# 1556174776/simple_pbft

Hardware: AMD Instinct MI355X
Metric: sig verifies/sec at 1/2/4/8 MI355X; p50 quorum-cert verify latency (higher is better)
Workload: dtype u32; 1 GPU; config4: 1048576 ECDSA-P256 sigs sharded N/1, 100-key table, 1% corrupted (8 classes); global_batch=1048576, keys=100, parallelism=shard1 (strong scaling: independent per-GPU shards, no collective), streams=2

## Files before the change

### simple_pbft_amd/csrc/kernels.h

```cpp
#pragma once
#include <hip/hip_runtime.h>
#include <stddef.h>
#include <stdint.h>

namespace pbftv {

size_t table_bytes(int w);
int table_windows(int w);
#define PBFTV_COMBOS_G29(X) X(29, 24) X(29, 22) X(29, 21) X(29, 20) X(29, 16)
#define PBFTV_COMBOS_G26(X) X(26, 24) X(26, 22) X(26, 21) X(26, 20) X(26, 16)
#define PBFTV_COMBOS_G24(X) X(24, 24) X(24, 22) X(24, 20) X(24, 16)
#define PBFTV_COMBOS_SMALL(X) X(20, 20) X(16, 16) X(16, 12) X(16, 8) X(8, 8)
#define PBFTV_COMBOS(X) PBFTV_COMBOS_G29(X) PBFTV_COMBOS_G26(X) PBFTV_COMBOS_G24(X) PBFTV_COMBOS_SMALL(X)
#define PBFTV_TABLE_WIDTHS(X) X(8) X(12) X(16) X(20) X(21) X(22) X(24) X(26) X(29)
struct TableScratch {
  void* bases;
  void* lbuf;
  void* hbuf;
  void* small_scratch;
  void* entry_scratch;
  uint64_t entry_lanes;
};
struct TableScratchSizes {
  size_t bases, lbuf, hbuf, small_scratch, entry_scratch;
  uint64_t entry_lanes;
};
TableScratchSizes table_scratch_sizes(int w, uint32_t nbases);
hipError_t launch_build_tables(int w, const uint32_t* keys_le, uint32_t key0, uint32_t nb, int with_g,
                               uint32_t* valid, uint32_t* const* tabs, TableScratch& sc, hipStream_t st);
size_t ecdsa_record_bytes(uint64_t n);
int scalar_batch(uint64_t n);
size_t scalar_prefix_bytes(uint64_t n);
struct KeyOrder {
  const uint32_t* total;
  uint32_t* claim;
  uint32_t nkeys;
};
hipError_t launch_ecdsa_scalars(const uint8_t* hashes, const uint8_t* sigs, const uint32_t* key_idx, uint64_t n,
                                const uint32_t* key_valid, uint32_t nkeys, void* rec, void* prefix,
                                const KeyOrder& ko, hipStream_t st);
hipError_t launch_ecdsa_comb(int wg, int wq, const void* rec, uint64_t n, const uint32_t* gtab,
                             const uint32_t* const* qtabs,
                             uint8_t* bitmap, uint8_t* okb, const uint32_t* cuflag, hipStream_t st);
constexpr uint32_t kCuFlagWords = 4096;
bool key_sort_wanted(uint64_t n, uint32_t nkeys);
size_t key_sort_header_bytes();
size_t key_sort_scratch_bytes(uint64_t n, uint32_t nkeys);
hipError_t launch_key_count(const uint32_t* key_idx, uint64_t n, uint32_t nkeys, void* scratch, uint32_t parity,
                            KeyOrder* out, hipStream_t st);
hipError_t launch_pack_bits(const uint8_t* okb, uint64_t n, uint8_t* bitmap, hipStream_t st);
struct CombArgs {
  const void* rec;
  uint64_t n;
  const uint32_t* gtab;
  const uint32_t* const* qtabs;
  uint8_t* bitmap;
  uint8_t* okb;
  const uint32_t* cuflag;
};
struct WaveArgs {
  const uint8_t* hashes;
  const uint8_t* sigs;
  const uint32_t* key_idx;
  uint64_t n;
  const uint32_t* key_valid;
  uint32_t nkeys;
  const uint32_t* gtab;
  const uint32_t* const* qtabs;
  uint8_t* bitmap;
  uint8_t* okbytes;
  bool one_wave;
};
hipError_t launch_ecdsa_wave(int wg, int wq, const uint8_t* hashes, const uint8_t* sigs, const uint32_t* key_idx,
                             uint64_t n, const uint32_t* key_valid, uint32_t nkeys, const uint32_t* gtab,
                             const uint32_t* const* qtabs, uint8_t* bitmap, uint8_t* okbytes, hipStream_t st,
                             bool one_wave = false);
uint64_t wave_path_max();
constexpr int kRowsExact = 4;

struct QcMail {
  uint32_t bell, n, stop, expired_s0, cap, halt, expired_s1, pad[9];
  static constexpr uint32_t kQcSlots = 8;
  static constexpr uint32_t kQcCap = 128;
  static constexpr int kArmSlots = 2;
  __host__ __device__ uint32_t* expired(int s) { return s ? &expired_s1 : &expired_s0; }
  static constexpr size_t slot_off(uint32_t i) { return 64 + 192 * (size_t)i; }
  static constexpr size_t live_off(int s = 0) { return 64 + 192 * (size_t)kQcSlots + 4 * (size_t)kQcCap * s; }
  static constexpr size_t res_off(uint32_t = kQcCap) { return live_off(kArmSlots); }
  static constexpr size_t arrays_off(uint32_t cap = kQcCap) {
    return (res_off() + (cap > kQcCap ? cap : kQcCap) + 63) & ~(size_t)63;
// ... 82 lines not shown
```

### simple_pbft_amd/csrc/p256_kernels.hip

```cpp
#include <hip/hip_runtime.h>

#include <cstdlib>

#include "kernels.h"
#include "verify_kernels.h"

namespace pbftv {

#ifndef PBFTV_SCAL_BLOCK_INV_MIN_K
#define PBFTV_SCAL_BLOCK_INV_MIN_K 4
#endif

#ifndef PBFTV_SCAL_WAVES
#define PBFTV_SCAL_WAVES 1
#endif

constexpr uint32_t kSortBlocks = 256;
constexpr uint32_t kSortMaxKeys = 1024;
constexpr uint32_t kSortHdr = kSortMaxKeys + 64;

template <int W>
struct TabGeom {
  using G = CombGeom<W>;
  static constexpr int CL = G::kEnt < 256 ? G::kEnt : (G::kW <= 16 ? 256 : 1 << (G::kW / 2));
// ... 245 lines not shown
  switch (w) {
#define PBFTV_W(W) \
  case W: return CombGeom<W>::kBytes;
    PBFTV_TABLE_WIDTHS(PBFTV_W)
#undef PBFTV_W
    default: return 0;
  }
}

int table_windows(int w) {
  switch (w) {
#define PBFTV_W(W) \
  case W: return CombGeom<W>::kWin;
    PBFTV_TABLE_WIDTHS(PBFTV_W)
#undef PBFTV_W
    default: return 0;
  }
}

hipError_t launch_build_tables(int w, const uint32_t* keys_le, uint32_t key0, uint32_t nb, int with_g,
                               uint32_t* valid, uint32_t* const* tabs, TableScratch& sc, hipStream_t st) {
  switch (w) {
#define PBFTV_W(W) \
  case W: return build_tables_w<W>(keys_le, key0, nb, with_g, valid, tabs, sc, st);
    PBFTV_TABLE_WIDTHS(PBFTV_W)
#undef PBFTV_W
    default: return hipErrorInvalidValue;
  }
}

__device__ __forceinline__ void block_key_hist(uint32_t* h, const uint32_t* __restrict__ key_idx, uint64_t n,
                                               uint32_t nkeys) {
  const uint32_t nb = nkeys + 1;
  for (uint32_t b = threadIdx.x; b < nb; b += blockDim.x) h[b] = 0;
  __syncthreads();
  const uint64_t chunk = (n + gridDim.x - 1) / gridDim.x, lo = (uint64_t)blockIdx.x * chunk;
  const uint64_t hi = lo + chunk < n ? lo + chunk : n;
  for (uint64_t i = lo + threadIdx.x; i < hi; i += blockDim.x) {
    const uint32_t k = key_idx[i];
    atomicAdd(&h[k < nkeys ? k : nkeys], 1u);
  }
  __syncthreads();
}

__global__ void __launch_bounds__(256) k_key_hist(const uint32_t* __restrict__ key_idx, uint64_t n, uint32_t nkeys,
                                                  uint32_t* __restrict__ cur, uint32_t* __restrict__ other) {
  __shared__ uint32_t h[kSortMaxKeys + 1];
  if (blockIdx.x == 0)
    for (uint32_t b = threadIdx.x; b < 2 * kSortHdr; b += blockDim.x) other[b] = 0;
  block_key_hist(h, key_idx, n, nkeys);
  for (uint32_t b = threadIdx.x; b <= nkeys; b += blockDim.x)
    if (h[b]) atomicAdd(&cur[b], h[b]);
}

__device__ __forceinline__ void block_key_starts(const uint32_t* __restrict__ total, uint32_t nkeys, uint32_t* start,
                                                 uint32_t* part) {
  constexpr uint32_t kPer = (kSortMaxKeys + 1 + 255) / 256;
  const uint32_t t = threadIdx.x, m = nkeys + 1;
  uint32_t v[kPer], sum = 0;
  PBFTV_UNROLL for (uint32_t k = 0; k < kPer; ++k) {
    const uint32_t b = kPer * t + k;
    v[k] = b < m ? total[b] : 0u;
    sum += v[k];
  }
  part[t] = sum;
  __syncthreads();
  for (uint32_t off = 1; off < 256; off <<= 1) {
    const uint32_t x = t >= off ? part[t - off] : 0u;
    __syncthreads();
    part[t] += x;
    __syncthreads();
  }
  uint32_t run = part[t] - sum;
  PBFTV_UNROLL for (uint32_t k = 0; k < kPer; ++k) {
    const uint32_t b = kPer * t + k;
    if (b < m) start[b] = run;
    run += v[k];
  }
  __syncthreads();
}

template <int K>
// ... 124 lines not shown
        if constexpr (kPre) {
          PBFTV_UNROLL for (int t = 0; t < 8; ++t) e[t] = pe[j][t];
        } else {
          load_be256(hashes + 32 * i, e);
        }
        fe ev, rv, t;
        fe_from_words(ev, e);
        fe_from_words(rv, r);
        fn_mul(t, ev, w);
        fn_canon(t, t);
        fe_to_words(u1, t);
        fn_mul(t, rv, w);
        fn_canon(t, t);
        fe_to_words(u2, t);
      }
      uint64_t at = i;
      uint32_t kj;
      if constexpr (kPre) kj = pk[j];
      else kj = key_idx[i];
      if (sorted) at = atomicAdd(&kh[kj < nk ? kj : nk], 1u);
      SigRec* o = rec + at;
      o->q[0] = make_uint4(u1[0], u1[1], u1[2], u1[3]);
      o->q[1] = make_uint4(u1[4], u1[5], u1[6], u1[7]);
      o->q[2] = make_uint4(u2[0], u2[1], u2[2], u2[3]);
      o->q[3] = make_uint4(u2[4], u2[5], u2[6], u2[7]);
      o->q[4] = make_uint4(r[0], r[1], r[2], r[3]);
      o->q[5] = make_uint4(r[4], r[5], r[6], r[7]);
      o->q[6] = make_uint4(ok ? kj : 0u, (uint32_t)i, ok ? 1u : 0u, 0u);
    }
  }
  PBFTV_SPROBE(5, okm);
}

__global__ void __launch_bounds__(256) k_pack_bits(const uint8_t* __restrict__ okb, uint64_t n,
                                                   uint8_t* __restrict__ bitmap) {
  const uint64_t b = (uint64_t)blockIdx.x * blockDim.x + threadIdx.x;
  if (8 * b >= n) return;
  uint32_t v = 0;
  if (8 * b + 8 <= n) {
    const uint2 w = *reinterpret_cast<const uint2*>(okb + 8 * b);
    PBFTV_UNROLL for (int k = 0; k < 4; ++k) v |= ((w.x >> (8 * k)) & 1u) << k;
    PBFTV_UNROLL for (int k = 0; k < 4; ++k) v |= ((w.y >> (8 * k)) & 1u) << (4 + k);
  } else {
    for (uint64_t k = 0; 8 * b + k < n; ++k) v |= (okb[8 * b + k] ? 1u : 0u) << k;
  }
  bitmap[b] = (uint8_t)v;
}

bool key_sort_wanted(uint64_t n, uint32_t nkeys) {
  if (const char* e = getenv("PBFTV_KEY_SORT")) {
    if (e[0] == '0') return false;
    if (e[0] == '1') return nkeys <= kSortMaxKeys && n < (1ull << 32);
  }
  return nkeys > 8 && nkeys <= kSortMaxKeys && n >= 32768 && n < (1ull << 32);
}

size_t key_sort_header_bytes() { return (size_t)(4 * kSortHdr) * 4; }
size_t key_sort_scratch_bytes(uint64_t, uint32_t) { return key_sort_header_bytes(); }

hipError_t launch_key_count(const uint32_t* key_idx, uint64_t n, uint32_t nkeys, void* scratch, uint32_t parity,
                            KeyOrder* out, hipStream_t st) {
  if (nkeys > kSortMaxKeys) return hipErrorInvalidValue;
  uint32_t* hdr = reinterpret_cast<uint32_t*>(scratch);
  uint32_t* cur = hdr + (parity & 1u) * 2 * kSortHdr;
  uint32_t* other = hdr + (~parity & 1u) * 2 * kSortHdr;
  *out = KeyOrder{cur, cur + kSortHdr, nkeys};
  if (n == 0) return hipSuccess;
  hipLaunchKernelGGL(k_key_hist, dim3(kSortBlocks), dim3(256), 0, st, key_idx, n, nkeys, cur, other);
  return hipGetLastError();
}

hipError_t launch_pack_bits(const uint8_t* okb, uint64_t n, uint8_t* bitmap, hipStream_t st) {
  if (n == 0) return hipSuccess;
  const uint64_t bytes = (n + 7) / 8;
  hipLaunchKernelGGL(k_pack_bits, dim3((uint32_t)((bytes + 255) / 256)), dim3(256), 0, st, okb, n, bitmap);
  return hipGetLastError();
}

bool launch_comb_part_g29(int wg, int wq, const CombArgs& a, hipStream_t st);
bool launch_comb_part_g26(int wg, int wq, const CombArgs& a, hipStream_t st);
bool launch_comb_part_g24(int wg, int wq, const CombArgs& a, hipStream_t st);
bool launch_comb_part_small(int wg, int wq, const CombArgs& a, hipStream_t st);
bool launch_wave_part_g29(int wg, int wq, const WaveArgs& a, hipStream_t st);
bool launch_wave_part_g26(int wg, int wq, const WaveArgs& a, hipStream_t st);
bool launch_wave_part_g24(int wg, int wq, const WaveArgs& a, hipStream_t st);
bool launch_wave_part_small(int wg, int wq, const WaveArgs& a, hipStream_t st);

hipError_t launch_ecdsa_wave(int wg, int wq, const uint8_t* hashes, const uint8_t* sigs, const uint32_t* key_idx,
                             uint64_t n, const uint32_t* key_valid, uint32_t nkeys, const uint32_t* gtab,
                             const uint32_t* const* qtabs, uint8_t* bitmap, uint8_t* okbytes, hipStream_t st,
                             bool one_wave) {
  if (n == 0) return hipSuccess;
  if (n > 0xFFFFFFFFull) return hipErrorInvalidValue;
  const WaveArgs a{hashes, sigs, key_idx, n, key_valid, nkeys, gtab, qtabs, bitmap, okbytes, one_wave};
  if (launch_wave_part_g29(wg, wq, a, st) || launch_wave_part_g26(wg, wq, a, st) ||
      launch_wave_part_g24(wg, wq, a, st) || launch_wave_part_small(wg, wq, a, st))
    return hipGetLastError();
  return hipErrorInvalidValue;
}

bool launch_armed_part_g29(int wg, int wq, const ArmArgs& a, hipStream_t st);
bool launch_armed_part_g26(int wg, int wq, const ArmArgs& a, hipStream_t st);
bool launch_armed_part_g24(int wg, int wq, const ArmArgs& a, hipStream_t st);
bool launch_armed_part_small(int wg, int wq, const ArmArgs& a, hipStream_t st);

hipError_t launch_ecdsa_wave_armed(int wg, int wq, const ArmArgs& a, hipStream_t st) {
  if (launch_armed_part_g29(wg, wq, a, st) || launch_armed_part_g26(wg, wq, a, st) ||
      launch_armed_part_g24(wg, wq, a, st) || launch_armed_part_small(wg, wq, a, st))
// ... 20 lines not shown
size_t scalar_prefix_bytes(uint64_t n) {
  const int k = scalar_batch(n);
  const uint64_t L = ((n + k - 1) / k + 255) / 256 * 256;
  return (size_t)k * 9 * L * 4;
}

template <int K>
static void launch_scalars_k(const uint8_t* hashes, const uint8_t* sigs, const uint32_t* key_idx, uint64_t n,
                             const uint32_t* key_valid, uint32_t nkeys, void* rec, uint32_t* prefix,
                             const KeyOrder& ko, hipStream_t st) {
  const uint64_t lanes = (n + K - 1) / K;
  const uint64_t blocks = (lanes + 255) / 256;
  hipLaunchKernelGGL(k_ecdsa_scalars<K>, dim3((uint32_t)blocks), dim3(256), 0, st, hashes, sigs, key_idx, n,
                     key_valid, nkeys, reinterpret_cast<SigRec*>(rec), prefix, ko);
}

hipError_t launch_ecdsa_scalars(const uint8_t* hashes, const uint8_t* sigs, const uint32_t* key_idx, uint64_t n,
                                const uint32_t* key_valid, uint32_t nkeys, void* rec, void* prefix,
                                const KeyOrder& ko, hipStream_t st) {
  if (n == 0) return hipSuccess;
  uint32_t* pf = reinterpret_cast<uint32_t*>(prefix);
  switch (scalar_batch(n)) {
    case 1: launch_scalars_k<1>(hashes, sigs, key_idx, n, key_valid, nkeys, rec, pf, ko, st); break;
    case 2: launch_scalars_k<2>(hashes, sigs, key_idx, n, key_valid, nkeys, rec, pf, ko, st); break;
    case 4: launch_scalars_k<4>(hashes, sigs, key_idx, n, key_valid, nkeys, rec, pf, ko, st); break;
    case 8: launch_scalars_k<8>(hashes, sigs, key_idx, n, key_valid, nkeys, rec, pf, ko, st); break;
    default: launch_scalars_k<16>(hashes, sigs, key_idx, n, key_valid, nkeys, rec, pf, ko, st); break;
  }
  return hipGetLastError();
}

hipError_t launch_ecdsa_comb(int wg, int wq, const void* rec, uint64_t n, const uint32_t* gtab,
                             const uint32_t* const* qtabs,
                             uint8_t* bitmap, uint8_t* okb, const uint32_t* cuflag, hipStream_t st) {
  if (n == 0) return hipSuccess;
  const CombArgs a{rec, n, gtab, qtabs, bitmap, okb, cuflag};
  if (launch_comb_part_g29(wg, wq, a, st) || launch_comb_part_g26(wg, wq, a, st) ||
      launch_comb_part_g24(wg, wq, a, st) || launch_comb_part_small(wg, wq, a, st))
    return hipGetLastError();
  return hipErrorInvalidValue;
}

size_t ecdsa_record_bytes(uint64_t n) { return (size_t)n * sizeof(SigRec); }

}

#ifdef PBFTV_SCAL_PROBE
extern "C" int pbftv_debug_scal_probe(uint64_t* out, size_t n) {
  return (int)hipMemcpyFromSymbol(out, HIP_SYMBOL(pbftv::g_scal_probe), n * sizeof(uint64_t), 0,
                                  hipMemcpyDeviceToHost);
}
#endif
```

### simple_pbft_amd/csrc/pbftv_api.cpp

```cpp
#include <hip/hip_runtime.h>

#include <algorithm>
#include <atomic>
#include <chrono>
#include <condition_variable>
#include <cstdio>
#include <cstdlib>
#include <cstring>
#include <functional>
#include <initializer_list>
#include <map>
#include <set>
#include <memory>
#include <mutex>
#include <string>
#include <thread>
#include <vector>

#include "../../include/pbftv.h"
#include "gojson.h"
#include "gojson_enc.h"
#include "kernels.h"

namespace {
// ... 107 lines not shown
  unsigned flags = hipHostMallocCoherent | hipHostMallocMapped;
  hipError_t ensure(size_t bytes) {
    if (bytes <= cap) return hipSuccess;
    if (p) {
      GpuQuiesce q(-1);
      (void)hipHostFree(p);
    }
    p = nullptr;
    cap = 0;
    size_t want = std::max<size_t>(bytes, 1 << 16);
    hipError_t e = hipHostMalloc(&p, want, flags);
    if (e == hipSuccess) cap = want;
    return e;
  }
  void release() {
    if (p) {
      GpuQuiesce q(-1);
      (void)hipHostFree(p);
    }
    p = nullptr;
    cap = 0;
  }
  HostBuf() = default;
  HostBuf(const HostBuf&) = delete;
  HostBuf& operator=(const HostBuf&) = delete;
  ~HostBuf() { release(); }
  template <class T>
  T* as() const {
    return reinterpret_cast<T*>(p);
  }
};

struct VerifyScratch {
  DevBuf rec, prefix, ksort, okb;
  uint32_t sort_parity = 0;
  void release() {
    rec.release();
    prefix.release();
    ksort.release();
    okb.release();
  }
};

struct Device {
  int id = -1;
  hipStream_t stream = nullptr;
  std::mutex mu;
  bool have_keys = false;
  bool mail_registered = false;
  bool keeper_stop = false, keeper_idle = false;
  bool qc_armed_served = false;
  HostBuf stage;
  std::atomic<uint32_t> arm_seq{0};
  uint32_t seq_counter = 0;
  int arm_stream = 1;
  uint32_t armed_first = 0;
  uint32_t retiring = 0;
  uint32_t arm_waves = 0;
  bool arm_wide = false;
  uint32_t qc_nmax = 0;
  uint32_t qc_nmax_prev = 0;
  uint32_t qc_slots = 4;
  uint32_t qc_wmax = 0;
  uint32_t qc_wslots = 0;
  bool arm_live = false;
  std::chrono::steady_clock::time_point last_wide{};
  std::chrono::steady_clock::time_point armed_at{}, last_qc{};
  uint64_t qc_ns_entry = 0, qc_ns_handover = 0, qc_ns_total = 0, qc_ns_slots = 0;
  char hot_end[1] = {};
  uint64_t qc_calls = 0, qc_armed = 0, qc_reruns = 0, qc_exact_sigs = 0, qc_launches = 0, qc_armings = 0;
  std::atomic<int64_t> busy_until_ns{0};
  std::shared_ptr<DevBuf> gtab;
  DevBuf key_valid, qptrs;
// ... 853 lines not shown
      }
      d->pending_frees.clear();
      for (void* p : d->pool_ptrs) (void)hipFreeAsync(p, d->astream);
      d->pool_ptrs.clear();
      (void)hipStreamSynchronize(d->astream);
      (void)hipMemPoolDestroy(d->pool);
      (void)hipStreamDestroy(d->astream);
    }
    for (hipEvent_t e : d->spare_ev) (void)hipEventDestroy(e);
    (void)hipStreamDestroy(d->stream);
  }
  if (!ctx->host_cache.empty()) {
    GpuQuiesce quiet(-1);
    for (auto& kv : ctx->host_cache) (void)hipHostFree(kv.second);
  }
  delete ctx;
}

int pbftv_device_count(const pbftv_ctx* ctx) { return ctx ? (int)ctx->devs.size() : 0; }

int pbftv_device_id(const pbftv_ctx* ctx, int i) {
  if (!ctx || i < 0 || i >= (int)ctx->devs.size()) return -1;
  return ctx->devs[i]->id;
}

int pbftv_reserve(pbftv_ctx* ctx, uint64_t n) {
  if (!ctx) return fail(PBFTV_EINVAL, "ctx is null");
  for (auto& dp : ctx->devs) {
    Device& d = *dp;
    std::lock_guard<std::mutex> lk(d.mu);
    HIP_TRY(hipSetDevice(d.id));
    HIP_TRY(d.vs.rec.ensure(pbftv::ecdsa_record_bytes(n)));
    HIP_TRY(d.vs.prefix.ensure(pbftv::scalar_prefix_bytes(n)));
    if (pbftv::key_sort_wanted(n, d.nkeys)) {
      HIP_TRY(ensure_key_sort(d.vs, n, d.nkeys, d.stream, true));
      HIP_TRY(d.vs.okb.ensure(n));
    }
  }
  return PBFTV_OK;
}

static Device* dev_of(pbftv_ctx* ctx, int dev) {
  if (!ctx || dev < 0 || dev >= (int)ctx->devs.size()) return nullptr;
  return ctx->devs[dev].get();
}

static hipError_t dev_pool_ready(Device& d) {
  if (d.pool) return hipSuccess;
  hipMemPoolProps props{};
  props.allocType = hipMemAllocationTypePinned;
  props.handleTypes = hipMemHandleTypeNone;
  props.location.type = hipMemLocationTypeDevice;
  props.location.id = d.id;
  HIP_TRY_E(hipMemPoolCreate(&d.pool, &props));
  uint64_t keep = UINT64_MAX;
  HIP_TRY_E(hipMemPoolSetAttribute(d.pool, hipMemPoolAttrReleaseThreshold, &keep));
  int no = 0;
  HIP_TRY_E(hipMemPoolSetAttribute(d.pool, hipMemPoolReuseAllowInternalDependencies, &no));
  HIP_TRY_E(hipMemPoolSetAttribute(d.pool, hipMemPoolReuseFollowEventDependencies, &no));
  HIP_TRY_E(hipStreamCreateWithFlags(&d.astream, hipStreamNonBlocking));
  return hipSuccess;
}

static hipError_t defer_free(Device& d, void* p) {
  if (d.scratch_st && d.scratch_st != d.stream && !d.stream_scratch.count(d.scratch_st) && d.scratch_ev)
    HIP_TRY_E(hipEventSynchronize(d.scratch_ev));
  for (auto& kv : d.reader_ev) HIP_TRY_E(hipEventSynchronize(kv.second));
  Device::PendingFree pf{p, {}};
  auto mark = [&](hipStream_t st) -> hipError_t {
    hipEvent_t e;
// ... 571 lines not shown
  for (auto& dp : ctx->devs) {
    const int64_t f = std::max<int64_t>(dp->busy_until_ns.load(std::memory_order_relaxed), now);
    if (f < best_free || (f == best_free && f <= now && dp->arm_seq.load(std::memory_order_relaxed) &&
                          !best->arm_seq.load(std::memory_order_relaxed))) {
      best = dp.get();
      best_free = f;
    }
  }
  return best;
}

static int verify_on_device(Device& d, const uint8_t* d_hashes, const uint8_t* d_sigs, const uint32_t* d_key_idx,
                            uint64_t n, uint8_t* d_bitmap, hipStream_t st, VerifyScratch* own = nullptr) {
  if (!d.have_keys) return fail(PBFTV_ENOKEYS, "pbftv_register_keys has not been called");
  if (n <= d.wave_max->load(std::memory_order_relaxed)) {
    HIP_TRY(timed(d, PBFTV_K_ECDSA_WAVE, st, [&] {
      return pbftv::launch_ecdsa_wave(d.gbits, d.qbits, d_hashes, d_sigs, d_key_idx, n, d.key_valid.as<uint32_t>(),
                                      d.nkeys, d.gtab->as<uint32_t>(), d.qptrs.as<const uint32_t* const>(), d_bitmap, nullptr, st);
    }));
    HIP_TRY(fence_reader(d, st));
    return PBFTV_OK;
  }
  if (!own) {
    auto it = d.stream_scratch.find(st);
    if (it != d.stream_scratch.end()) own = it->second.get();
  }
  VerifyScratch& sc = own ? *own : d.vs;
  note_busy(d, n);
  HIP_TRY(sc.rec.ensure(pbftv::ecdsa_record_bytes(n)));
  HIP_TRY(sc.prefix.ensure(pbftv::scalar_prefix_bytes(n)));
  if (!own) HIP_TRY(scratch_acquire(d, st));
  const bool sorted = pbftv::key_sort_wanted(n, d.nkeys);
  pbftv::KeyOrder ko{nullptr, nullptr, 0};
  if (sorted) {
    HIP_TRY(sc.okb.ensure(n));
    HIP_TRY(ensure_key_sort(sc, n, d.nkeys, st));
    HIP_TRY(pbftv::launch_key_count(d_key_idx, n, d.nkeys, sc.ksort.p, sc.sort_parity++, &ko, st));
  }
  HIP_TRY(timed(d, PBFTV_K_ECDSA_SCALARS, st, [&] {
    return pbftv::launch_ecdsa_scalars(d_hashes, d_sigs, d_key_idx, n, d.key_valid.as<uint32_t>(), d.nkeys, sc.rec.p,
                                       sc.prefix.p, ko, st);
  }));
  HIP_TRY(timed(d, PBFTV_K_ECDSA_COMB, st, [&] {
    return pbftv::launch_ecdsa_comb(d.gbits, d.qbits, sc.rec.p, n, d.gtab->as<uint32_t>(),
                                    d.qptrs.as<const uint32_t* const>(), d_bitmap,
                                    sorted ? sc.okb.as<uint8_t>() : nullptr,
                                    qc_cu_yield() && d.arm_seq.load(std::memory_order_relaxed)
                                        ? d.cuflag_ready.load(std::memory_order_acquire)
                                        : nullptr,
                                    st);
  }));
  if (sorted) HIP_TRY(pbftv::launch_pack_bits(sc.okb.as<uint8_t>(), n, d_bitmap, st));
  if (!own) HIP_TRY(scratch_release(d, st));
  return PBFTV_OK;
}

static bool env_flag(const char* name, bool dflt) {
  const char* e = getenv(name);
  return e ? e[0] == '1' : dflt;
}

static uint64_t host_chunk() {
  uint64_t c = 262144;
  if (const char* e = getenv("PBFTV_HOST_CHUNK")) c = std::max<uint64_t>(512, strtoull(e, nullptr, 10));
  return (c + 511) / 512 * 512;
}

static std::vector<uint64_t> host_chunks(uint64_t m) {
  const uint64_t c = host_chunk();
  uint64_t last = 131072;
  if (const char* e = getenv("PBFTV_HOST_LAST")) last = strtoull(e, nullptr, 10) / 512 * 512;
  if (last >= c || m <= c) last = 0;
  const uint64_t head = last ? (m - last) / 512 * 512 : m;
  std::vector<uint64_t> out;
  for (uint64_t r = head; r > 0; r -= std::min(c, r)) out.push_back(std::min(c, r));
  if (m > head) out.push_back(m - head);
  return out;
}

static int host_slots() {
  int s = Device::kSlots;
  if (const char* e = getenv("PBFTV_HOST_SLOTS")) s = atoi(e);
  return std::min(Device::kSlots, std::max(2, s));
}

// ... 936 lines not shown
```

### simple_pbft_amd/csrc/verify_kernels.h

```cpp
#pragma once
#include <hip/hip_runtime.h>

#include <type_traits>

#include "kernels.h"
#include "p256_algo.h"
#include "rows.h"

namespace pbftv {

#ifndef PBFTV_COMB_BLOCK
#define PBFTV_COMB_BLOCK 256
#endif

#ifndef PBFTV_COMB_WAVES
#define PBFTV_COMB_WAVES 4
#endif

#ifdef PBFTV_SCAL_PROBE
static __device__ uint64_t g_scal_probe[8192 * 8];
#define PBFTV_SPROBE(k, dep)                                                            \
  do {                                                                                  \
    asm volatile("" ::"v"(dep));                                                        \
    const uint64_t t_ = wall_clock64();                                                 \
// ... 165 lines not shown
  asm volatile("s_waitcnt vmcnt(0)" ::: "memory");
  uint4 e[4];
  PBFTV_UNROLL for (int k = 0; k < 4; ++k) e[k] = sent[k][t];
  entry_words(e, ew);
}


constexpr uint64_t kCuParkTicks = 5000;
__device__ __forceinline__ uint32_t cu_flag_index() {
  uint32_t hw, xcc;
  asm volatile("s_getreg_b32 %0, hwreg(HW_REG_HW_ID)" : "=s"(hw));
  asm volatile("s_getreg_b32 %0, hwreg(HW_REG_XCC_ID)" : "=s"(xcc));
  return ((xcc & 15u) << 8) | ((hw >> 8) & 0xFFu);
}
__device__ __forceinline__ void raise_cu_flags(uint32_t* f, uint32_t* f2) {
  if (f && (threadIdx.x & 63u) == 0) {
    __hip_atomic_fetch_add(f, 1u, __ATOMIC_RELAXED, __HIP_MEMORY_SCOPE_AGENT);
    if (f2) __hip_atomic_fetch_add(f2, 1u, __ATOMIC_RELAXED, __HIP_MEMORY_SCOPE_AGENT);
  }
}
__device__ __forceinline__ void comb_park(const uint32_t* f) {
  const uint64_t t0 = wall_clock64();
  do {
    __builtin_amdgcn_s_sleep(4);
  } while (__builtin_amdgcn_readfirstlane(__hip_atomic_load(f, __ATOMIC_RELAXED, __HIP_MEMORY_SCOPE_AGENT)) != 0 &&
           wall_clock64() - t0 < kCuParkTicks);
}

template <int WG, int WQ>
__global__ void __launch_bounds__(PBFTV_COMB_BLOCK, PBFTV_COMB_WAVES) k_ecdsa_comb(const SigRec* __restrict__ rec, uint64_t n,
                                                                    const uint4* __restrict__ gtab,
                                                                    const uint4* const* __restrict__ qtabs,
                                                                    uint8_t* __restrict__ bitmap,
                                                                    uint8_t* __restrict__ okb,
                                                                    const uint32_t* __restrict__ cuflag) {
  using S = CombSteps<WG, WQ>;
  __shared__ typename S::Digit sdig[S::nD][PBFTV_COMB_BLOCK];
  __shared__ uint4 sent[4][PBFTV_COMB_BLOCK];
  const uint32_t t = threadIdx.x;
  const uint32_t nb = gridDim.x, b = blockIdx.x, per = nb / 8;
  const uint32_t blk = b < 8 * per ? (b % 8) * per + b / 8 : b;
  const uint64_t p = (uint64_t)blk * blockDim.x + t;
  const SigRec* rp = rec + p;
  uint4 meta = make_uint4(0, 0, 0, 0);
  if (p < n) meta = rp->q[6];
  bool ok = false;
  const bool act = meta.z != 0;
  {
    uint4 a = make_uint4(0, 0, 0, 0), b = a, c = a, dd = a;
    if (act) {
      a = rp->q[0];
      b = rp->q[1];
      c = rp->q[2];
      dd = rp->q[3];
    }
    const uint32_t w1[8] = {a.x, a.y, a.z, a.w, b.x, b.y, b.z, b.w};
    const uint32_t w2[8] = {c.x, c.y, c.z, c.w, dd.x, dd.y, dd.z, dd.w};
    digit_cut<WG> s1;
    digit_cut<WQ> s2;
    PBFTV_UNROLL for (int j = 0; j < S::nD; ++j)
      sdig[j][t] = (typename S::Digit)((S::is_q(j) ? s2.at(w2, S::win(j)) : s1.at(w1, S::win(j))) - 1);
  }
  const uint4* qtab = act ? qtabs[meta.x] : gtab;
  xyzz_s R;
  bool inf = true, neg_y = false;
  const int d0 = (int)sdig[0][t] + 1, d1 = (int)sdig[1][t] + 1;
  const bool first2 = __ballot(act && (d0 == 0 || d1 == 0)) == 0;
// ... 21 lines not shown
    j0 = 0;
  }
  const int jend = fuse ? S::nD - 1 : S::nD;
#ifndef PBFTV_COMB_UNROLL
#define PBFTV_COMB_UNROLL 1
#endif
  const uint32_t* cuf = cuflag ? cuflag + cu_flag_index() : nullptr;
#pragma unroll PBFTV_COMB_UNROLL
  for (int j = j0; j < jend; ++j) {
    uint32_t w16[16];
    read_entry_lds(sent, t, w16);
    const int dc = d;
    const uint32_t cf = cuf ? __hip_atomic_load(cuf, __ATOMIC_RELAXED, __HIP_MEMORY_SCOPE_AGENT) : 0u;
    if (j + 1 < S::nD) {
      d = (int)sdig[j + 1][t] + 1;
      issue_entry_lds(sent, t, S::is_q(j + 1) ? entry_ptr<WQ>(qtab, S::win(j + 1), d)
                                              : entry_ptr<WG>(gtab, S::win(j + 1), d));
    }
    comb_step_s(R, inf, neg_y, dc, w16);
    if (cuf && __builtin_amdgcn_readfirstlane(cf) != 0) comb_park(cuf);
  }
  if (act) {
    const uint4 e = rp->q[4], f = rp->q[5];
    const uint32_t r[8] = {e.x, e.y, e.z, e.w, f.x, f.y, f.z, f.w};
    int res;
    if (fuse) {
      uint32_t w16[16];
      read_entry_lds(sent, t, w16);
      res = comb_last_check_s(R, neg_y, d, w16, r);
    } else {
      res = (!inf && fs_is_zero(R.zz)) ? -1 : (ecdsa_check(R, !inf, r) ? 1 : 0);
    }
    ok = res < 0 ? comb2_checked_verify<WG, WQ>(rp, gtab, qtab) : res == 1;
  }
  if (okb != nullptr) {
    if (p < n) okb[meta.y] = ok ? 1 : 0;
    return;
  }
  const unsigned long long m = __ballot(ok);
  const uint32_t lane = t & 63u;
  const uint64_t wave_base = p - lane;
  if (lane < 8 && wave_base + 8 * lane < n) bitmap[(wave_base >> 3) + lane] = (uint8_t)(m >> (8 * lane));
}

__device__ __forceinline__ void shfl_xor_fe(fe& dst, const fe& src, int m) {
  PBFTV_UNROLL for (int l = 0; l < 9; ++l) dst.v[l] = (uint32_t)__shfl_xor((int)src.v[l], m, 64);
}

__device__ __forceinline__ void jac_add_complete(jac& r, bool& rinf, const jac& p, bool pinf, const jac& q,
                                                 bool qinf) {
  if (pinf || qinf) {
    r = pinf ? q : p;
    rinf = pinf && qinf;
    return;
  }
  jac s;
  const int st = jac_add(s, p, q);
  if (st == 1) {
    jac_double(r, p);
    rinf = false;
  } else {
    r = s;
    rinf = st == 2;
  }
}

template <int WG, int WQ>
__device__ __forceinline__ void wave_sum_lanes(jac& P, bool& inf, const uint32_t u1[8], const uint32_t u2[8],
                                               const uint4* __restrict__ gtab, const uint4* __restrict__ qtab) {
// ... 1251 lines not shown
      attr = true;
    }
  }
  hipLaunchKernelGGL((k_ecdsa_wave_armed<WG, WQ>), dim3((a.relay ? QcMail::kQcCap : QcMail::kQcSlots) / 4), dim3(256), lds,
                     st, a);
}

template <int WG, int WQ>
void launch_wave_w(const uint8_t* hashes, const uint8_t* sigs, const uint32_t* key_idx, uint64_t n,
                          const uint32_t* key_valid, uint32_t nkeys, const uint32_t* gtab,
                          const uint32_t* const* qtabs,
                          uint8_t* bitmap, uint8_t* okbytes, hipStream_t st, bool one_wave = false) {
  if constexpr (RowsGeom<WG, WQ>::ok) {
    if (n <= rows_max_batch() && rows_enabled() && !one_wave) {
      hipLaunchKernelGGL((k_ecdsa_rows<WG, WQ>), dim3((uint32_t)n), dim3(64 * RowsGeom<WG, WQ>::waves), 0, st, hashes, sigs, key_idx,
                         n, key_valid, nkeys, reinterpret_cast<const uint4*>(gtab),
                         reinterpret_cast<const uint4* const*>(qtabs), bitmap, okbytes);
      return;
    }
  }
  if (one_wave) {
    hipLaunchKernelGGL((k_ecdsa_wave_lean<WG, WQ>), dim3((uint32_t)n), dim3(64), 0, st, hashes, sigs, key_idx, n,
                       key_valid, nkeys, reinterpret_cast<const uint4*>(gtab),
                       reinterpret_cast<const uint4* const*>(qtabs), bitmap, okbytes);
    return;
  }
  hipLaunchKernelGGL((k_ecdsa_wave<WG, WQ>), dim3((uint32_t)n), dim3(64), 0, st, hashes, sigs, key_idx, n, key_valid,
                     nkeys, reinterpret_cast<const uint4*>(gtab), reinterpret_cast<const uint4* const*>(qtabs), bitmap,
                     okbytes);
}

template <int WG, int WQ>
void launch_comb_w(const void* rec, uint64_t n, const uint32_t* gtab, const uint32_t* const* qtabs, uint8_t* bitmap,
                   uint8_t* okb, const uint32_t* cuflag, hipStream_t st) {
  const uint64_t blocks = (n + PBFTV_COMB_BLOCK - 1) / PBFTV_COMB_BLOCK;
  hipLaunchKernelGGL((k_ecdsa_comb<WG, WQ>), dim3((uint32_t)blocks), dim3(PBFTV_COMB_BLOCK), 0, st,
                     reinterpret_cast<const SigRec*>(rec), n, reinterpret_cast<const uint4*>(gtab),
                     reinterpret_cast<const uint4* const*>(qtabs), bitmap, okb, cuflag);
}

#define PBFTV_VERIFY_PART(NAME, COMBOS)                                                                       \
  bool launch_comb_part_##NAME(int wg, int wq, const CombArgs& a, hipStream_t st) {                           \
    COMBOS(PBFTV_PART_COMB_CASE)                                                                              \
    return false;                                                                                             \
  }                                                                                                           \
  bool launch_wave_part_##NAME(int wg, int wq, const WaveArgs& a, hipStream_t st) {                           \
    COMBOS(PBFTV_PART_WAVE_CASE)                                                                              \
    return false;                                                                                             \
  }                                                                                                           \
  bool launch_armed_part_##NAME(int wg, int wq, const ArmArgs& a, hipStream_t st) {                           \
    COMBOS(PBFTV_PART_ARMED_CASE)                                                                             \
    return false;                                                                                             \
  }
#define PBFTV_PART_COMB_CASE(G, Q)                                                                            \
  if (wg == G && wq == Q) {                                                                                   \
    launch_comb_w<G, Q>(a.rec, a.n, a.gtab, a.qtabs, a.bitmap, a.okb, a.cuflag, st);                                    \
    return true;                                                                                              \
  }
#define PBFTV_PART_ARMED_CASE(G, Q)                                                                           \
  if (wg == G && wq == Q) {                                                                                   \
    launch_armed_w<G, Q>(a, st);                                                                              \
    return true;                                                                                              \
  }
#define PBFTV_PART_WAVE_CASE(G, Q)                                                                            \
  if (wg == G && wq == Q) {                                                                                   \
    launch_wave_w<G, Q>(a.hashes, a.sigs, a.key_idx, a.n, a.key_valid, a.nkeys, a.gtab, a.qtabs, a.bitmap,    \
                        a.okbytes, st, a.one_wave);                                                           \
    return true;                                                                                              \
  }

}
```

Baseline: 924.1 million verifies/s.

## Scatter verify results directly into bitmap via atomics, dropping pack-bits pass

```diff
diff --git a/simple_pbft_amd/csrc/kernels.h b/simple_pbft_amd/csrc/kernels.h
--- a/simple_pbft_amd/csrc/kernels.h
+++ b/simple_pbft_amd/csrc/kernels.h
@@ -41,21 +41,20 @@
                                 const KeyOrder& ko, hipStream_t st);
 hipError_t launch_ecdsa_comb(int wg, int wq, const void* rec, uint64_t n, const uint32_t* gtab,
                              const uint32_t* const* qtabs,
-                             uint8_t* bitmap, uint8_t* okb, const uint32_t* cuflag, hipStream_t st);
+                             uint8_t* bitmap, bool key_order, const uint32_t* cuflag, hipStream_t st);
 constexpr uint32_t kCuFlagWords = 4096;
 bool key_sort_wanted(uint64_t n, uint32_t nkeys);
 size_t key_sort_header_bytes();
 size_t key_sort_scratch_bytes(uint64_t n, uint32_t nkeys);
 hipError_t launch_key_count(const uint32_t* key_idx, uint64_t n, uint32_t nkeys, void* scratch, uint32_t parity,
-                            KeyOrder* out, hipStream_t st);
-hipError_t launch_pack_bits(const uint8_t* okb, uint64_t n, uint8_t* bitmap, hipStream_t st);
+                            uint8_t* bitmap, KeyOrder* out, hipStream_t st);
 struct CombArgs {
   const void* rec;
   uint64_t n;
   const uint32_t* gtab;
   const uint32_t* const* qtabs;
   uint8_t* bitmap;
-  uint8_t* okb;
+  bool key_order;
   const uint32_t* cuflag;
 };
 struct WaveArgs {
diff --git a/simple_pbft_amd/csrc/p256_kernels.hip b/simple_pbft_amd/csrc/p256_kernels.hip
--- a/simple_pbft_amd/csrc/p256_kernels.hip
+++ b/simple_pbft_amd/csrc/p256_kernels.hip
@@ -303,20 +303,54 @@
   const uint32_t nb = nkeys + 1;
   for (uint32_t b = threadIdx.x; b < nb; b += blockDim.x) h[b] = 0;
   __syncthreads();
-  const uint64_t chunk = (n + gridDim.x - 1) / gridDim.x, lo = (uint64_t)blockIdx.x * chunk;
-  const uint64_t hi = lo + chunk < n ? lo + chunk : n;
-  for (uint64_t i = lo + threadIdx.x; i < hi; i += blockDim.x) {
-    const uint32_t k = key_idx[i];
-    atomicAdd(&h[k < nkeys ? k : nkeys], 1u);
+  auto count = [&](uint32_t k) { atomicAdd(&h[k < nkeys ? k : nkeys], 1u); };
+  constexpr int kHistLoads = 4;
+  const uint64_t to16 = ((16u - (uint32_t)(reinterpret_cast<uintptr_t>(key_idx) & 15u)) & 15u) >> 2;
+  const uint64_t head = to16 < n ? to16 : n;
+  const uint64_t nv = (n - head) >> 2, tail0 = head + 4 * nv;
+  const uint4* __restrict__ v = reinterpret_cast<const uint4*>(key_idx + head);
+  const uint64_t stride = (uint64_t)gridDim.x * blockDim.x;
+  for (uint64_t i = (uint64_t)blockIdx.x * blockDim.x + threadIdx.x; i < nv; i += kHistLoads * stride) {
+    uint4 q[kHistLoads];
+    PBFTV_UNROLL for (int k = 0; k < kHistLoads; ++k)
+      if (i + k * stride < nv) q[k] = v[i + k * stride];
+    PBFTV_UNROLL for (int k = 0; k < kHistLoads; ++k)
+      if (i + k * stride < nv) {
+        count(q[k].x);
+        count(q[k].y);
+        count(q[k].z);
+        count(q[k].w);
+      }
+  }
+  if (blockIdx.x == 0) {
+    const uint64_t t = threadIdx.x;
+    if (t < head) count(key_idx[t]);
+    else if (tail0 + (t - head) < n) count(key_idx[tail0 + (t - head)]);
   }
   __syncthreads();
 }
 
+__device__ __forceinline__ void grid_zero_bytes(uint8_t* __restrict__ bm, uint64_t bytes) {
+  const uint64_t to4 = (4u - (uint32_t)(reinterpret_cast<uintptr_t>(bm) & 3u)) & 3u;
+  const uint64_t head = to4 < bytes ? to4 : bytes;
+  const uint64_t nw = (bytes - head) >> 2, tail0 = head + 4 * nw;
+  uint32_t* __restrict__ w = reinterpret_cast<uint32_t*>(bm + head);
+  const uint64_t stride = (uint64_t)gridDim.x * blockDim.x;
+  for (uint64_t i = (uint64_t)blockIdx.x * blockDim.x + threadIdx.x; i < nw; i += stride) w[i] = 0;
+  if (blockIdx.x == gridDim.x - 1) {
+    const uint64_t t = threadIdx.x;
+    if (t < head) bm[t] = 0;
+    else if (tail0 + (t - head) < bytes) bm[tail0 + (t - head)] = 0;
+  }
+}
+
 __global__ void __launch_bounds__(256) k_key_hist(const uint32_t* __restrict__ key_idx, uint64_t n, uint32_t nkeys,
-                                                  uint32_t* __restrict__ cur, uint32_t* __restrict__ other) {
+                                                  uint32_t* __restrict__ cur, uint32_t* __restrict__ other,
+                                                  uint8_t* __restrict__ bitmap) {
   __shared__ uint32_t h[kSortMaxKeys + 1];
   if (blockIdx.x == 0)
     for (uint32_t b = threadIdx.x; b < 2 * kSortHdr; b += blockDim.x) other[b] = 0;
+  grid_zero_bytes(bitmap, (n + 7) / 8);
   block_key_hist(h, key_idx, n, nkeys);
   for (uint32_t b = threadIdx.x; b <= nkeys; b += blockDim.x)
     if (h[b]) atomicAdd(&cur[b], h[b]);
@@ -507,21 +541,6 @@
   PBFTV_SPROBE(5, okm);
 }
 
-__global__ void __launch_bounds__(256) k_pack_bits(const uint8_t* __restrict__ okb, uint64_t n,
-                                                   uint8_t* __restrict__ bitmap) {
-  const uint64_t b = (uint64_t)blockIdx.x * blockDim.x + threadIdx.x;
-  if (8 * b >= n) return;
-  uint32_t v = 0;
-  if (8 * b + 8 <= n) {
-    const uint2 w = *reinterpret_cast<const uint2*>(okb + 8 * b);
-    PBFTV_UNROLL for (int k = 0; k < 4; ++k) v |= ((w.x >> (8 * k)) & 1u) << k;
-    PBFTV_UNROLL for (int k = 0; k < 4; ++k) v |= ((w.y >> (8 * k)) & 1u) << (4 + k);
-  } else {
-    for (uint64_t k = 0; 8 * b + k < n; ++k) v |= (okb[8 * b + k] ? 1u : 0u) << k;
-  }
-  bitmap[b] = (uint8_t)v;
-}
-
 bool key_sort_wanted(uint64_t n, uint32_t nkeys) {
   if (const char* e = getenv("PBFTV_KEY_SORT")) {
     if (e[0] == '0') return false;
@@ -534,21 +553,15 @@
 size_t key_sort_scratch_bytes(uint64_t, uint32_t) { return key_sort_header_bytes(); }
 
 hipError_t launch_key_count(const uint32_t* key_idx, uint64_t n, uint32_t nkeys, void* scratch, uint32_t parity,
-                            KeyOrder* out, hipStream_t st) {
+                            uint8_t* bitmap, KeyOrder* out, hipStream_t st) {
   if (nkeys > kSortMaxKeys) return hipErrorInvalidValue;
   uint32_t* hdr = reinterpret_cast<uint32_t*>(scratch);
   uint32_t* cur = hdr + (parity & 1u) * 2 * kSortHdr;
   uint32_t* other = hdr + (~parity & 1u) * 2 * kSortHdr;
   *out = KeyOrder{cur, cur + kSortHdr, nkeys};
   if (n == 0) return hipSuccess;
-  hipLaunchKernelGGL(k_key_hist, dim3(kSortBlocks), dim3(256), 0, st, key_idx, n, nkeys, cur, other);
-  return hipGetLastError();
-}
-
-hipError_t launch_pack_bits(const uint8_t* okb, uint64_t n, uint8_t* bitmap, hipStream_t st) {
-  if (n == 0) return hipSuccess;
-  const uint64_t bytes = (n + 7) / 8;
-  hipLaunchKernelGGL(k_pack_bits, dim3((uint32_t)((bytes + 255) / 256)), dim3(256), 0, st, okb, n, bitmap);
+  hipLaunchKernelGGL(k_key_hist, dim3(kSortBlocks), dim3(256), 0, st, key_idx, n, nkeys, cur, other,
+                     bitmap);
   return hipGetLastError();
 }
 
@@ -635,9 +648,9 @@
 
 hipError_t launch_ecdsa_comb(int wg, int wq, const void* rec, uint64_t n, const uint32_t* gtab,
                              const uint32_t* const* qtabs,
-                             uint8_t* bitmap, uint8_t* okb, const uint32_t* cuflag, hipStream_t st) {
+                             uint8_t* bitmap, bool key_order, const uint32_t* cuflag, hipStream_t st) {
   if (n == 0) return hipSuccess;
-  const CombArgs a{rec, n, gtab, qtabs, bitmap, okb, cuflag};
+  const CombArgs a{rec, n, gtab, qtabs, bitmap, key_order, cuflag};
   if (launch_comb_part_g29(wg, wq, a, st) || launch_comb_part_g26(wg, wq, a, st) ||
       launch_comb_part_g24(wg, wq, a, st) || launch_comb_part_small(wg, wq, a, st))
     return hipGetLastError();
diff --git a/simple_pbft_amd/csrc/pbftv_api.cpp b/simple_pbft_amd/csrc/pbftv_api.cpp
--- a/simple_pbft_amd/csrc/pbftv_api.cpp
+++ b/simple_pbft_amd/csrc/pbftv_api.cpp
@@ -163,13 +163,12 @@
 };
 
 struct VerifyScratch {
-  DevBuf rec, prefix, ksort, okb;
+  DevBuf rec, prefix, ksort;
   uint32_t sort_parity = 0;
   void release() {
     rec.release();
     prefix.release();
     ksort.release();
-    okb.release();
   }
 };
 
@@ -1089,10 +1088,7 @@
     HIP_TRY(hipSetDevice(d.id));
     HIP_TRY(d.vs.rec.ensure(pbftv::ecdsa_record_bytes(n)));
     HIP_TRY(d.vs.prefix.ensure(pbftv::scalar_prefix_bytes(n)));
-    if (pbftv::key_sort_wanted(n, d.nkeys)) {
-      HIP_TRY(ensure_key_sort(d.vs, n, d.nkeys, d.stream, true));
-      HIP_TRY(d.vs.okb.ensure(n));
-    }
+    if (pbftv::key_sort_wanted(n, d.nkeys)) HIP_TRY(ensure_key_sort(d.vs, n, d.nkeys, d.stream, true));
   }
   return PBFTV_OK;
 }
@@ -1731,9 +1727,8 @@
   const bool sorted = pbftv::key_sort_wanted(n, d.nkeys);
   pbftv::KeyOrder ko{nullptr, nullptr, 0};
   if (sorted) {
-    HIP_TRY(sc.okb.ensure(n));
     HIP_TRY(ensure_key_sort(sc, n, d.nkeys, st));
-    HIP_TRY(pbftv::launch_key_count(d_key_idx, n, d.nkeys, sc.ksort.p, sc.sort_parity++, &ko, st));
+    HIP_TRY(pbftv::launch_key_count(d_key_idx, n, d.nkeys, sc.ksort.p, sc.sort_parity++, d_bitmap, &ko, st));
   }
   HIP_TRY(timed(d, PBFTV_K_ECDSA_SCALARS, st, [&] {
     return pbftv::launch_ecdsa_scalars(d_hashes, d_sigs, d_key_idx, n, d.key_valid.as<uint32_t>(), d.nkeys, sc.rec.p,
@@ -1741,14 +1736,12 @@
   }));
   HIP_TRY(timed(d, PBFTV_K_ECDSA_COMB, st, [&] {
     return pbftv::launch_ecdsa_comb(d.gbits, d.qbits, sc.rec.p, n, d.gtab->as<uint32_t>(),
-                                    d.qptrs.as<const uint32_t* const>(), d_bitmap,
-                                    sorted ? sc.okb.as<uint8_t>() : nullptr,
+                                    d.qptrs.as<const uint32_t* const>(), d_bitmap, sorted,
                                     qc_cu_yield() && d.arm_seq.load(std::memory_order_relaxed)
                                         ? d.cuflag_ready.load(std::memory_order_acquire)
                                         : nullptr,
                                     st);
   }));
-  if (sorted) HIP_TRY(pbftv::launch_pack_bits(sc.okb.as<uint8_t>(), n, d_bitmap, st));
   if (!own) HIP_TRY(scratch_release(d, st));
   return PBFTV_OK;
 }
diff --git a/simple_pbft_amd/csrc/verify_kernels.h b/simple_pbft_amd/csrc/verify_kernels.h
--- a/simple_pbft_amd/csrc/verify_kernels.h
+++ b/simple_pbft_amd/csrc/verify_kernels.h
@@ -221,7 +221,7 @@
                                                                     const uint4* __restrict__ gtab,
                                                                     const uint4* const* __restrict__ qtabs,
                                                                     uint8_t* __restrict__ bitmap,
-                                                                    uint8_t* __restrict__ okb,
+                                                                    uint32_t key_order,
                                                                     const uint32_t* __restrict__ cuflag) {
   using S = CombSteps<WG, WQ>;
   __shared__ typename S::Digit sdig[S::nD][PBFTV_COMB_BLOCK];
@@ -310,8 +310,13 @@
     }
     ok = res < 0 ? comb2_checked_verify<WG, WQ>(rp, gtab, qtab) : res == 1;
   }
-  if (okb != nullptr) {
-    if (p < n) okb[meta.y] = ok ? 1 : 0;
+  if (key_order) {
+    if (ok) {
+      uint8_t* byte = bitmap + (meta.y >> 3);
+      const uint32_t in_word = (uint32_t)(reinterpret_cast<uintptr_t>(byte) & 3);
+      (void)__hip_atomic_fetch_or(reinterpret_cast<uint32_t*>(byte - in_word), 1u << (8 * in_word + (meta.y & 7u)),
+                                  __ATOMIC_RELAXED, __HIP_MEMORY_SCOPE_AGENT);
+    }
     return;
   }
   const unsigned long long m = __ballot(ok);
@@ -1629,11 +1634,11 @@
 
 template <int WG, int WQ>
 void launch_comb_w(const void* rec, uint64_t n, const uint32_t* gtab, const uint32_t* const* qtabs, uint8_t* bitmap,
-                   uint8_t* okb, const uint32_t* cuflag, hipStream_t st) {
+                   bool key_order, const uint32_t* cuflag, hipStream_t st) {
   const uint64_t blocks = (n + PBFTV_COMB_BLOCK - 1) / PBFTV_COMB_BLOCK;
   hipLaunchKernelGGL((k_ecdsa_comb<WG, WQ>), dim3((uint32_t)blocks), dim3(PBFTV_COMB_BLOCK), 0, st,
                      reinterpret_cast<const SigRec*>(rec), n, reinterpret_cast<const uint4*>(gtab),
-                     reinterpret_cast<const uint4* const*>(qtabs), bitmap, okb, cuflag);
+                     reinterpret_cast<const uint4* const*>(qtabs), bitmap, key_order ? 1u : 0u, cuflag);
 }
 
 #define PBFTV_VERIFY_PART(NAME, COMBOS)                                                                       \
@@ -1651,7 +1656,7 @@
   }
 #define PBFTV_PART_COMB_CASE(G, Q)                                                                            \
   if (wg == G && wq == Q) {                                                                                   \
-    launch_comb_w<G, Q>(a.rec, a.n, a.gtab, a.qtabs, a.bitmap, a.okb, a.cuflag, st);                                    \
+    launch_comb_w<G, Q>(a.rec, a.n, a.gtab, a.qtabs, a.bitmap, a.key_order, a.cuflag, st);                   \
     return true;                                                                                              \
   }
 #define PBFTV_PART_ARMED_CASE(G, Q)                                                                           \
```

Measured after the change: 931.4 million verifies/s (median of 6 runs). About the same (+0.8%).

## Write verify bits directly into bitmap from comb kernel; vectorize key histogram

Applied to the files above, without the earlier changes.

```diff
diff --git a/simple_pbft_amd/csrc/kernels.h b/simple_pbft_amd/csrc/kernels.h
--- a/simple_pbft_amd/csrc/kernels.h
+++ b/simple_pbft_amd/csrc/kernels.h
@@ -41,7 +41,8 @@
                                 const KeyOrder& ko, hipStream_t st);
 hipError_t launch_ecdsa_comb(int wg, int wq, const void* rec, uint64_t n, const uint32_t* gtab,
                              const uint32_t* const* qtabs,
-                             uint8_t* bitmap, uint8_t* okb, const uint32_t* cuflag, hipStream_t st);
+                             uint8_t* bitmap, uint8_t* okb, bool by_index, const uint32_t* cuflag, hipStream_t st);
+bool comb_bitmap_direct(uint64_t n, const void* bitmap);
 constexpr uint32_t kCuFlagWords = 4096;
 bool key_sort_wanted(uint64_t n, uint32_t nkeys);
 size_t key_sort_header_bytes();
@@ -56,6 +57,7 @@
   const uint32_t* const* qtabs;
   uint8_t* bitmap;
   uint8_t* okb;
+  bool by_index;
   const uint32_t* cuflag;
 };
 struct WaveArgs {
diff --git a/simple_pbft_amd/csrc/p256_kernels.hip b/simple_pbft_amd/csrc/p256_kernels.hip
--- a/simple_pbft_amd/csrc/p256_kernels.hip
+++ b/simple_pbft_amd/csrc/p256_kernels.hip
@@ -301,13 +301,36 @@
 __device__ __forceinline__ void block_key_hist(uint32_t* h, const uint32_t* __restrict__ key_idx, uint64_t n,
                                                uint32_t nkeys) {
   const uint32_t nb = nkeys + 1;
-  for (uint32_t b = threadIdx.x; b < nb; b += blockDim.x) h[b] = 0;
+  const uint32_t t = threadIdx.x;
+  for (uint32_t b = t; b < nb; b += blockDim.x) h[b] = 0;
   __syncthreads();
-  const uint64_t chunk = (n + gridDim.x - 1) / gridDim.x, lo = (uint64_t)blockIdx.x * chunk;
-  const uint64_t hi = lo + chunk < n ? lo + chunk : n;
-  for (uint64_t i = lo + threadIdx.x; i < hi; i += blockDim.x) {
-    const uint32_t k = key_idx[i];
-    atomicAdd(&h[k < nkeys ? k : nkeys], 1u);
+  const uint64_t mis = (reinterpret_cast<uintptr_t>(key_idx) >> 2) & 3u;
+  const uint64_t head = mis ? (4 - mis < n ? 4 - mis : n) : 0;
+  const uint64_t nv = (n - head) >> 2, tail0 = head + 4 * nv;
+  const uint4* __restrict__ body = reinterpret_cast<const uint4*>(key_idx + head);
+  const uint64_t chunk = (nv + gridDim.x - 1) / gridDim.x, lo = (uint64_t)blockIdx.x * chunk;
+  const uint64_t hi = lo + chunk < nv ? lo + chunk : nv;
+  constexpr int kT = 4;
+  for (uint64_t v0 = lo + t; v0 < hi; v0 += (uint64_t)kT * blockDim.x) {
+    uint4 k[kT];
+    PBFTV_UNROLL for (int j = 0; j < kT; ++j) {
+      const uint64_t v = v0 + (uint64_t)j * blockDim.x;
+      k[j] = body[v < hi ? v : hi - 1];
+    }
+    PBFTV_UNROLL for (int j = 0; j < kT; ++j) {
+      const uint32_t one = v0 + (uint64_t)j * blockDim.x < hi ? 1u : 0u;
+      atomicAdd(&h[k[j].x < nkeys ? k[j].x : nkeys], one);
+      atomicAdd(&h[k[j].y < nkeys ? k[j].y : nkeys], one);
+      atomicAdd(&h[k[j].z < nkeys ? k[j].z : nkeys], one);
+      atomicAdd(&h[k[j].w < nkeys ? k[j].w : nkeys], one);
+    }
+  }
+  if (blockIdx.x == 0 && t < 8) {
+    const uint64_t i = t < 4 ? t : tail0 + (t - 4);
+    if (t < 4 ? i < head : i < n) {
+      const uint32_t k = key_idx[i];
+      atomicAdd(&h[k < nkeys ? k : nkeys], 1u);
+    }
   }
   __syncthreads();
 }
@@ -530,6 +553,12 @@
   return nkeys > 8 && nkeys <= kSortMaxKeys && n >= 32768 && n < (1ull << 32);
 }
 
+bool comb_bitmap_direct(uint64_t n, const void* bitmap) {
+  if (const char* e = getenv("PBFTV_COMB_BITMAP"))
+    if (e[0] == '0') return false;
+  return n % 32 == 0 && reinterpret_cast<uintptr_t>(bitmap) % 4 == 0;
+}
+
 size_t key_sort_header_bytes() { return (size_t)(4 * kSortHdr) * 4; }
 size_t key_sort_scratch_bytes(uint64_t, uint32_t) { return key_sort_header_bytes(); }
 
@@ -635,9 +664,10 @@
 
 hipError_t launch_ecdsa_comb(int wg, int wq, const void* rec, uint64_t n, const uint32_t* gtab,
                              const uint32_t* const* qtabs,
-                             uint8_t* bitmap, uint8_t* okb, const uint32_t* cuflag, hipStream_t st) {
+                             uint8_t* bitmap, uint8_t* okb, bool by_index, const uint32_t* cuflag, hipStream_t st) {
   if (n == 0) return hipSuccess;
-  const CombArgs a{rec, n, gtab, qtabs, bitmap, okb, cuflag};
+  if (by_index && (n % 32 != 0 || reinterpret_cast<uintptr_t>(bitmap) % 4 != 0)) return hipErrorInvalidValue;
+  const CombArgs a{rec, n, gtab, qtabs, bitmap, okb, by_index, cuflag};
   if (launch_comb_part_g29(wg, wq, a, st) || launch_comb_part_g26(wg, wq, a, st) ||
       launch_comb_part_g24(wg, wq, a, st) || launch_comb_part_small(wg, wq, a, st))
     return hipGetLastError();
diff --git a/simple_pbft_amd/csrc/pbftv_api.cpp b/simple_pbft_amd/csrc/pbftv_api.cpp
--- a/simple_pbft_amd/csrc/pbftv_api.cpp
+++ b/simple_pbft_amd/csrc/pbftv_api.cpp
@@ -1091,7 +1091,7 @@
     HIP_TRY(d.vs.prefix.ensure(pbftv::scalar_prefix_bytes(n)));
     if (pbftv::key_sort_wanted(n, d.nkeys)) {
       HIP_TRY(ensure_key_sort(d.vs, n, d.nkeys, d.stream, true));
-      HIP_TRY(d.vs.okb.ensure(n));
+      if (n % 32 != 0) HIP_TRY(d.vs.okb.ensure(n));
     }
   }
   return PBFTV_OK;
@@ -1730,8 +1730,9 @@
   if (!own) HIP_TRY(scratch_acquire(d, st));
   const bool sorted = pbftv::key_sort_wanted(n, d.nkeys);
   pbftv::KeyOrder ko{nullptr, nullptr, 0};
+  const bool direct = sorted && pbftv::comb_bitmap_direct(n, d_bitmap);
   if (sorted) {
-    HIP_TRY(sc.okb.ensure(n));
+    if (!direct) HIP_TRY(sc.okb.ensure(n));
     HIP_TRY(ensure_key_sort(sc, n, d.nkeys, st));
     HIP_TRY(pbftv::launch_key_count(d_key_idx, n, d.nkeys, sc.ksort.p, sc.sort_parity++, &ko, st));
   }
@@ -1742,13 +1743,13 @@
   HIP_TRY(timed(d, PBFTV_K_ECDSA_COMB, st, [&] {
     return pbftv::launch_ecdsa_comb(d.gbits, d.qbits, sc.rec.p, n, d.gtab->as<uint32_t>(),
                                     d.qptrs.as<const uint32_t* const>(), d_bitmap,
-                                    sorted ? sc.okb.as<uint8_t>() : nullptr,
+                                    sorted && !direct ? sc.okb.as<uint8_t>() : nullptr, direct,
                                     qc_cu_yield() && d.arm_seq.load(std::memory_order_relaxed)
                                         ? d.cuflag_ready.load(std::memory_order_acquire)
                                         : nullptr,
                                     st);
   }));
-  if (sorted) HIP_TRY(pbftv::launch_pack_bits(sc.okb.as<uint8_t>(), n, d_bitmap, st));
+  if (sorted && !direct) HIP_TRY(pbftv::launch_pack_bits(sc.okb.as<uint8_t>(), n, d_bitmap, st));
   if (!own) HIP_TRY(scratch_release(d, st));
   return PBFTV_OK;
 }
diff --git a/simple_pbft_amd/csrc/verify_kernels.h b/simple_pbft_amd/csrc/verify_kernels.h
--- a/simple_pbft_amd/csrc/verify_kernels.h
+++ b/simple_pbft_amd/csrc/verify_kernels.h
@@ -222,6 +222,7 @@
                                                                     const uint4* const* __restrict__ qtabs,
                                                                     uint8_t* __restrict__ bitmap,
                                                                     uint8_t* __restrict__ okb,
+                                                                    uint32_t by_index,
                                                                     const uint32_t* __restrict__ cuflag) {
   using S = CombSteps<WG, WQ>;
   __shared__ typename S::Digit sdig[S::nD][PBFTV_COMB_BLOCK];
@@ -309,6 +310,15 @@
       res = (!inf && fs_is_zero(R.zz)) ? -1 : (ecdsa_check(R, !inf, r) ? 1 : 0);
     }
     ok = res < 0 ? comb2_checked_verify<WG, WQ>(rp, gtab, qtab) : res == 1;
+  }
+  if (by_index) {
+    if (p < n) {
+      unsigned int* word = reinterpret_cast<unsigned int*>(bitmap) + (meta.y >> 5);
+      const unsigned int bit = 1u << (meta.y & 31u);
+      if (ok) atomicOr(word, bit);
+      else atomicAnd(word, ~bit);
+    }
+    return;
   }
   if (okb != nullptr) {
     if (p < n) okb[meta.y] = ok ? 1 : 0;
@@ -1629,11 +1639,11 @@
 
 template <int WG, int WQ>
 void launch_comb_w(const void* rec, uint64_t n, const uint32_t* gtab, const uint32_t* const* qtabs, uint8_t* bitmap,
-                   uint8_t* okb, const uint32_t* cuflag, hipStream_t st) {
+                   uint8_t* okb, bool by_index, const uint32_t* cuflag, hipStream_t st) {
   const uint64_t blocks = (n + PBFTV_COMB_BLOCK - 1) / PBFTV_COMB_BLOCK;
   hipLaunchKernelGGL((k_ecdsa_comb<WG, WQ>), dim3((uint32_t)blocks), dim3(PBFTV_COMB_BLOCK), 0, st,
                      reinterpret_cast<const SigRec*>(rec), n, reinterpret_cast<const uint4*>(gtab),
-                     reinterpret_cast<const uint4* const*>(qtabs), bitmap, okb, cuflag);
+                     reinterpret_cast<const uint4* const*>(qtabs), bitmap, okb, by_index ? 1u : 0u, cuflag);
 }
 
 #define PBFTV_VERIFY_PART(NAME, COMBOS)                                                                       \
@@ -1651,7 +1661,7 @@
   }
 #define PBFTV_PART_COMB_CASE(G, Q)                                                                            \
   if (wg == G && wq == Q) {                                                                                   \
-    launch_comb_w<G, Q>(a.rec, a.n, a.gtab, a.qtabs, a.bitmap, a.okb, a.cuflag, st);                                    \
+    launch_comb_w<G, Q>(a.rec, a.n, a.gtab, a.qtabs, a.bitmap, a.okb, a.by_index, a.cuflag, st);              \
     return true;                                                                                              \
   }
 #define PBFTV_PART_ARMED_CASE(G, Q)                                                                           \
```

New measurement: 933.9 million verifies/s before, 942.2 million verifies/s after, median of 6. No clear change (+0.9%).
